# luoao-kddi/SCP

Hardware: AMD Instinct MI355X
Metric: KITTI frames/sec encode (SCP-EHEM, level 16) + bpp match vs ref (higher is better)
Workload: dtype f32 (dense layers and attention as bf16x3 split on bf16 MFMA, feature kNN as f16x3 split on f16 MFMA, fp32 accumulate; position kNN / CDF in fp32); 1 GPU; SCP-EHEM KITTI-like synthetic 120k-pt frames, --spher --mullevel lidar_level=16 (BASELINE.json configs[2]), seeded random weights; nodes_per_frame=577403, windows_per_frame=100, frames_per_gpu=46, frames_in_flight=4, frames_per_launch_sequence=1, transform=host-numpy on a prefetch thread (strict identity: the reference's integers), parallelism=frame-sharded x1, rank_cores=256, rank_cores_pinned=False

## Files before the change

include/scp.h:

```cpp
#ifndef SCP_H
#define SCP_H
#include <stddef.h>
#include <stdint.h>

#ifdef __cplusplus
extern "C" {
#endif

#define SCP_API __attribute__((visibility("default")))

#define SCP_OK 0
#define SCP_EINVAL (-1)
#define SCP_ENOMEM (-2)
#define SCP_ESMALL (-3)
#define SCP_EHIP (-4)
#define SCP_ESTATE (-5)

#define SCP_MAX_DEPTH 21
#define SCP_MAX_SEGMENTS 62

#define SCP_ABI_VERSION 220
SCP_API int scp_version(void);
SCP_API int scp_last_hip_error(void);
SCP_API int scp_device_count(void);
// ... 260 lines not shown
typedef struct scp_expand_seg {
    int64_t first, count, cfirst, coded;
    int32_t L, shift, lv_next, lv_clamp, polar, reserved;
    double mn, den;
} scp_expand_seg;
SCP_API int scp_decode_expand_batch(const int64_t *sym, const int64_t *cum, const int32_t *pos, const uint8_t *anc, const uint8_t *octant,
                                    int64_t n, const scp_expand_seg *seg, int32_t S, int32_t cs, const int64_t *wbase, int32_t K, int64_t M,
                                    int64_t T, void *table_dev, int32_t *cpos, uint8_t *canc, uint8_t *coct, uint8_t *cctx, float *cposn,
                                    uint8_t *occ8, void *stream);

SCP_API int scp_swin_ln_linear(const float *x, int64_t ldx, const float *valid, const void *Whi, const void *Wlo, const float *bias,
                               const float *wbeta, float eps, float *out, int64_t ldo, int32_t M, int32_t N, void *stream);
SCP_API int scp_swin_post_attn(const void *Ohi, const void *Olo, int64_t ldo_in, const float *x, int64_t ldx, const void *W, const float *bp,
                               const float *b1, const float *b2, float eps, float *out, int64_t ldc, int32_t M, const int32_t *tile_list,
                               int32_t n_tiles, void *stream);
SCP_API int64_t scp_swin_post_attn_weight_bytes(void);
SCP_API double scp_gelu_prescale(void);

SCP_API int scp_swin_merge(const float *x, int64_t ldx, int64_t n_src, const int64_t *ia, const int64_t *ib, const void *W, const float *wbeta,
                           float eps, float *out, int64_t ldo, int32_t M, void *stream);

SCP_API int scp_geo_edge_mlps(const float *pos1, int64_t ld1, const float *pos2, int64_t ld2, const float *pos3, int64_t ld3, const void *W,
                              const float *bias, float *out, int64_t ldo, int32_t M, void *stream);
SCP_API int scp_mlp3_rows(const float *x, int64_t ldx, int64_t n_src, const int64_t *in_map, const void *W, const float *bias, float *out, int64_t ldo,
                          const int64_t *out_map, int32_t M, int32_t N, void *stream);

SCP_API int scp_swin_kv_planes(const float *k, const float *v, int64_t ldkv, int64_t rows, void *khi, void *klo, void *vthi, void *vtlo, void *stream);
SCP_API int scp_swin_ln_qkv(const float *x, int64_t ldx, const float *valid, const void *Whi, const void *Wlo, const float *bias, const float *wbeta,
                            float eps, float *q, int64_t ldq, void *planes, int64_t Tp, int32_t M, int32_t N, void *stream);
SCP_API int scp_swin_attention_packed_planes(const float *q, const void *khi, const void *klo, const void *vthi, const void *vtlo,
// ... 8 lines not shown
```

scp_amd/csrc/rc_common.h:

```cpp
#pragma once
#include "scp_internal.h"

typedef __bf16 rbf16x8 __attribute__((ext_vector_type(8)));
typedef float rf32x16 __attribute__((ext_vector_type(16)));
typedef float rf32x4 __attribute__((ext_vector_type(4)));
typedef int ri32x4 __attribute__((ext_vector_type(4)));
typedef __attribute__((address_space(3))) void *rc_lds_ptr_t;
typedef const __attribute__((address_space(1))) void *rc_glb_ptr_t;

#define RC_ROWS 128
#define RC_BOUNCE 4096

__device__ __forceinline__ void rc_dma16(const void *g, char *l) {
    __builtin_amdgcn_global_load_lds((rc_glb_ptr_t)g, (rc_lds_ptr_t)l, 16, 0, 0);
}

typedef float rf32x2 __attribute__((ext_vector_type(2)));
typedef __bf16 rbf16x2 __attribute__((ext_vector_type(2)));
typedef unsigned ru32x4 __attribute__((ext_vector_type(4)));
typedef unsigned ru32x2 __attribute__((ext_vector_type(2)));
__device__ __forceinline__ unsigned rc_pack2(float a, float b) {
    const rf32x2 v = {a, b};
    return __builtin_bit_cast(unsigned, __builtin_convertvector(v, rbf16x2));
}
__device__ __forceinline__ void rc_split2(float a, float b, unsigned &hi, unsigned &lo) {
    asm volatile("" : "+v"(a), "+v"(b));
    hi = rc_pack2(a, b);
    lo = rc_pack2(a - __builtin_bit_cast(float, hi << 16), b - __builtin_bit_cast(float, hi & 0xffff0000u));
}
__device__ __forceinline__ void rc_split8(const float *f, rbf16x8 &hi, rbf16x8 &lo) {
    ru32x4 h, l;
#pragma unroll
    for (int i = 0; i < 4; ++i) { unsigned a, b; rc_split2(f[2 * i], f[2 * i + 1], a, b); h[i] = a; l[i] = b; }
    hi = __builtin_bit_cast(rbf16x8, h);
    lo = __builtin_bit_cast(rbf16x8, l);
}

struct RcLane {
    int lane, col, h, w;
    int frag;
    int rg;
};

// ... 57 lines not shown
```

scp_amd/csrc/rowchain.hip:

```cpp
#include <stdlib.h>
#include "scp_internal.h"
#include "rc_common.h"

#define RC_SLOT 32768
#define RC_RING (4 * RC_SLOT)
#define RC_OFF_BOUNCE RC_RING
#define RC_OFF_BIAS (RC_RING + 4 * RC_BOUNCE)
#define RC_LDS (RC_OFF_BIAS + 16384)

__device__ __forceinline__ void rc_issue_rowchunk(const RcLane &L, const __bf16 *Whi, const __bf16 *Wlo, int g, char *slot) {
#pragma unroll
    for (int j = 0; j < 4; ++j) {
        const int p = L.w + 4 * j;
        const int64_t off = ((int64_t)g * 16 + p) * 512 + L.lane * 8;
        rc_dma16(Whi + off, slot + p * 1024);
        rc_dma16(Wlo + off, slot + 16384 + p * 1024);
    }
}

__device__ __forceinline__ void rc_issue_kchunk(const RcLane &L, const __bf16 *Whi, const __bf16 *Wlo, int c, int nks, char *slot) {
#pragma unroll
    for (int j = 0; j < 4; ++j) {
        const int p = L.w + 4 * j;
        const int64_t off = ((int64_t)p * nks + c) * 512 + L.lane * 8;
// ... 556 lines not shown
            if (RC_DMA_HERE(s, gap) && RC_PROBE_DMA_ON) rc_dma_piece(L, wr, RC_DMA_SLOT(s, gap) ? n1 : n0, nxt + RC_DMA_SLOT(s, gap) * RC_SLOT, RC_DMA_IDX(s, gap), RC_DMA_PLANE(s, gap));
            if (HAS_GELU) {
                const int k = s >> 1, st = (s & 1) * 6 + gap;
                unsigned wh = 0, wl = 0;
                rc_gelu_stage(st, g, a1g[2 * k], a1g[2 * k + 1], wh, wl);
                if (st == 10) Hnh[k >> 2][k & 3] = wh;
                if (st == 11) Hnl[k >> 2][k & 3] = wl;
            }
            RC_SB;
        }
    }
    if (NEXT == 0) RC_DS_READ4_WAIT(A[0][1], fn.r0, 16384, A[0][3], fn.k0, RC_SLOT + 16384, A[0][0], fn.r0, 0, A[0][2], fn.k0, RC_SLOT);
    else RC_DS_READ4_WAIT(A[0][1], fn.r0, 16384, A[0][3], fn.r0, RC_SLOT + 16384, A[0][0], fn.r0, 0, A[0][2], fn.r0, RC_SLOT);
}

__global__ __launch_bounds__(256, 1) void rc_post_attn_kernel(const RcPostArgs a) {
    extern __shared__ __attribute__((aligned(1024))) char smem[];
    const RcLane L = rc_lane();
    const int ntiles = (a.M + RC_ROWS - 1) / RC_ROWS;
    float *sbp = (float *)(smem + RC_OFF_BIAS), *sb2 = sbp + 256, *sb1 = sbp + 512;
    for (int i = threadIdx.x; i < 256; i += 256) { sbp[i] = a.bp[i]; sb2[i] = a.b2[i]; }
    for (int i = threadIdx.x; i < 1024; i += 256) sb1[i] = a.b1[i];
    __syncthreads();
    const int nlist = a.tile_list ? a.n_list : ntiles;
    auto tile_of = [&](int i) { return a.tile_list ? a.tile_list[i] : i; };
    int ti = blockIdx.x;
    if (ti >= nlist) return;
    int tile = tile_of(ti);
    char *bounce = smem + RC_OFF_BOUNCE + L.w * RC_BOUNCE;
    const int ldc_bytes = (int)(a.ldc * 4);
    const int voff = (32 * L.w + (L.lane >> 3)) * ldc_bytes + (L.lane & 7) * 16;
// ... 190 lines not shown
        load_o(tile_next);
        rc_body_step<false, true, 0>(L, smem, gstep & 1, Y, a1[0], a1[1], Hh[0], Hl[0], Hnh, Hnl, Bh, Bl, A, wr, src_2(31), src_2(31));
        ++gstep;
        rc_body_step<false, false, 1>(L, smem, gstep & 1, Y, a1[0], a1[1], Hnh, Hnl, Hh[0], Hl[0], Bh, Bl, A, wr, src_p(0), src_p(1));
        ++gstep;
        }
        stamp(t_mlp);
        asm volatile("s_waitcnt lgkmcnt(0)" ::: "memory");
        const int64_t rows_left = (int64_t)a.M - m0;
        const int64_t span = (rows_left < RC_ROWS ? rows_left : RC_ROWS) * a.ldc * 4;
#ifdef RC_EPI_NOSTORE
        const __amdgpu_buffer_rsrc_t rs = __builtin_amdgcn_make_buffer_rsrc(a.out, 0, 0, 0x00020000);
#else
        const __amdgpu_buffer_rsrc_t rs = __builtin_amdgcn_make_buffer_rsrc(a.out + (int64_t)m0 * a.ldc, 0, (int)span, 0x00020000);
#endif
#pragma unroll
        for (int b = 0; b < 8; ++b) {
            rf32x4 o[4];
#pragma unroll
            for (int q = 0; q < 4; ++q)
#pragma unroll
                for (int u = 0; u < 4; ++u) o[q][u] = Y[b][4 * q + u];
            rc_store_block(L, bounce, o, rs, ldc_bytes, voff, 32 * b);
        }
        transpose_o();
        stamp(t_epi);
        ++n_tiles;
    }
    if (DBG && L.lane == 0) {
        unsigned long long *o = a.dbg + ((size_t)blockIdx.x * 4 + L.w) * 8;
        o[0] = t_p0; o[1] = t_mlp; o[2] = t_ln; o[3] = t_epi; o[4] = n_tiles;
        o[5] = __builtin_amdgcn_s_memtime() - t_first; o[6] = __builtin_amdgcn_s_memrealtime() - r_first;
    }
    SCP_WAIT_DMA(0);
}

#ifndef RCW_D1
#define RCW_D1 4
// ... 684 lines not shown
        configured = true;
    }
    RcLnLinArgs a;
    a.x = x; a.ldx = ldx; a.valid = valid; a.Whi = (const __bf16 *)Whi; a.Wlo = (const __bf16 *)Wlo; a.bias = bias; a.wbeta = wbeta;
    a.out = q; a.ldo = q ? ldq : 256; a.M = M; a.N = N; a.eps = eps; a.probe = 0; a.dbg = nullptr;
    a.planes = (__bf16 *)planes; a.plane_bytes = Tp * 512; a.nq = N / 64 - 8;
    const int ntiles = M / RC_ROWS, ncu = rc_num_cu();
    SCP_PROF(SCP_PROF_LN_LINEAR, stream, 2.0 * M * 256.0 * N);
    if (rc_lnlin2_here(ntiles, ncu)) return scp_lnlin2_launch(a, true, ncu, (hipStream_t)stream);
    a.ngroups = rc_ll_groups(ntiles, N / 64, ncu);
    hipLaunchKernelGGL((rc_ln_linear_kernel<0, true>), dim3((unsigned)(a.ngroups > 1 ? ntiles * a.ngroups : (ntiles < ncu ? ntiles : ncu))), dim3(256), RC_LDS, (hipStream_t)stream, a);
    LAUNCH_CHECK();
    return SCP_OK;
}

extern "C" SCP_API int scp_swin_post_attn(const void *Ohi, const void *Olo, int64_t ldo_in, const float *x, int64_t ldx, const void *W, const float *bp,
                                          const float *b1, const float *b2, float eps, float *out, int64_t ldc, int32_t M, const int32_t *tile_list,
                                          int32_t n_tiles, void *stream) {
    if (!Ohi || !Olo || !x || !W || !bp || !b1 || !b2 || !out || M <= 0 || (tile_list && (n_tiles <= 0 || n_tiles > (M + RC_ROWS - 1) / RC_ROWS)) || ldo_in < 256 || (ldo_in & 7) || ldx < 256 || (ldx & 3) || ldc < 256 ||
        (ldc & 3) || (((uintptr_t)Ohi | (uintptr_t)Olo | (uintptr_t)x | (uintptr_t)out | (uintptr_t)W) & 15) ||
        (int64_t)RC_ROWS * ldc * 4 > 0x7fffffffLL)
        return SCP_EINVAL;
    static bool configured = false;
    if (!configured) {
        HIP_TRY(hipFuncSetAttribute((const void *)rc_post_attn_kernel, hipFuncAttributeMaxDynamicSharedMemorySize, RC_LDS));
        HIP_TRY(hipFuncSetAttribute((const void *)rc_post_attn_wide_kernel, hipFuncAttributeMaxDynamicSharedMemorySize, RC_LDS));
        configured = true;
    }
    RcPostArgs a;
    a.Ohi = (const __bf16 *)Ohi; a.Olo = (const __bf16 *)Olo; a.ldo_in = ldo_in; a.x = x; a.ldx = ldx; a.W = W;
    a.bp = bp; a.b1 = b1; a.b2 = b2; a.out = out; a.ldc = ldc; a.M = M; a.eps = eps;
    a.dbg = g_rc_dbg;
    { const char *e = getenv("SCP_RC_DUMP"); a.dbg_mode = e ? atoi(e) : 0; }
    a.tile_list = tile_list; a.n_list = tile_list ? n_tiles : 0;
    const int ntiles = tile_list ? n_tiles : (M + RC_ROWS - 1) / RC_ROWS;
    const int ncu = rc_num_cu();
    SCP_PROF(SCP_PROF_POST_ATTN, stream, 2.0 * (tile_list ? (double)n_tiles * RC_ROWS : (double)M) * (256.0 * 256.0 + 2.0 * 256.0 * 1024.0));
    if (rc_wide_mode() == 1 || (rc_wide_mode() < 0 && !g_rc_dbg && !a.dbg_mode && 4 * (int64_t)ntiles <= (int64_t)ncu)) {
        const int items = 4 * ntiles;
        hipLaunchKernelGGL(rc_post_attn_wide_kernel, dim3((unsigned)(items < 2 * ncu ? items : 2 * ncu)), dim3(256), RC_LDS, (hipStream_t)stream, a);
        LAUNCH_CHECK();
        return SCP_OK;
    }
    hipLaunchKernelGGL(rc_post_attn_kernel, dim3((unsigned)(ntiles < ncu ? ntiles : ncu)), dim3(256), RC_LDS, (hipStream_t)stream, a);
    LAUNCH_CHECK();
    return SCP_OK;
}

extern "C" SCP_API int64_t scp_swin_post_attn_weight_bytes(void) { return 2 * (int64_t)RC_W_PLANE; }

extern "C" SCP_API int scp_geo_edge_mlps(const float *pos1, int64_t ld1, const float *pos2, int64_t ld2, const float *pos3, int64_t ld3, const void *W,
                                         const float *bias, float *out, int64_t ldo, int32_t M, void *stream) {
    if (!pos1 || !pos2 || !pos3 || !W || !bias || !out || M <= 0 || ld1 < 64 || ld2 < 128 || ld3 < 256 || ((ld1 | ld2 | ld3) & 3) || ldo < 128 || (ldo & 3) ||
        (((uintptr_t)pos1 | (uintptr_t)pos2 | (uintptr_t)pos3 | (uintptr_t)out | (uintptr_t)W) & 15) || (int64_t)RC_ROWS * ldo * 4 > 0x7fffffffLL)
        return SCP_EINVAL;
    static bool configured = false;
    if (!configured) {
        HIP_TRY(hipFuncSetAttribute((const void *)rc_edge_mlp_kernel, hipFuncAttributeMaxDynamicSharedMemorySize, RC_LDS));
        configured = true;
    }
    RcEdgeArgs a;
// ... 46 lines not shown
```

scp_amd/models/packed.py:

```python
import numpy as np
import torch
import torch.nn.functional as F

from .. import native
from ..ops import linear_s, leaky_mlp3_s, split_cat, linear, layer_norm, leaky_mlp3, _split, derived, frozen_epoch
from .ehem import SHIFT, WINDOW, _edge_conv_packed, qkv_fused


def _ceil512(a):
    return (a + WINDOW - 1) // WINDOW * WINDOW


def _tokens(L):
    wid = torch.repeat_interleave(torch.arange(L.numel(), device=L.device), L)
    first = torch.cumsum(L, 0) - L
    return wid, torch.arange(int(L.sum()), device=L.device) - first[wid]


class StageLayout:

    def __init__(self, L):
        self.L = L
        self.Lp = _ceil512(L)
        self.base = torch.cumsum(self.Lp, 0) - self.Lp
# ... 104 lines not shown


def _block_consts(layer, cross):
    ep = frozen_epoch()
    key = "_scp_fast_x" if cross else "_scp_fast"
    fast = layer.__dict__.get(key) if ep else None
    if fast is not None and fast[0] == ep:
        return fast[1:]
    att = layer.attention.self
    out = (_rowchain_weights(layer, cross), att.relative_position_bias_table, (att.query.bias if cross else None), layer.layernorm_before.eps, layer.layernorm_after.eps)
    if ep:
        layer.__dict__[key] = (ep,) + out
    return out


def _swin_layer_rowchain(layer, x, valid, wtab, shift, query=None, tiles=None, q_pre=None):
    cross = query is not None
    w, table, qbias, eps_b, eps_a = _block_consts(layer, cross)
    v1 = None if valid is None else valid.reshape(-1)
    if native.attention_bf16x3():
        if not cross:
            q, kvp = native.swin_ln_qkv(x, w["kv"], w["b"], eps_b, v1)
        else:
            q = q_pre if q_pre is not None else native.swin_ln_linear(query, w["q"], qbias, eps_b, v1)
            _, kvp = native.swin_ln_qkv(x, w["kv"], w["b"], eps_b, v1)
        o = native.swin_attention_packed_planes(q, kvp, table, wtab, shift, split=True, valid=v1 if tiles is not None else None)
        if tiles is not None and tiles.shape[0] > 0:
            return native.swin_post_attn(o, x, w["post"], eps_a, out=x, tiles=tiles)
        return native.swin_post_attn(o, x, w["post"], eps_a)
    att, lnb = layer.attention.self, layer.layernorm_before
    if not cross:
        qkv = native.swin_ln_linear(x, w["kv"], w["b"], lnb.eps, v1)
        q, k, v = qkv[:, :256], qkv[:, 256:512], qkv[:, 512:]
    else:
        q = q_pre if q_pre is not None else native.swin_ln_linear(query, w["q"], att.query.bias, lnb.eps, v1)
        kv = native.swin_ln_linear(x, w["kv"], w["b"], lnb.eps, v1)
        k, v = kv[:, :256], kv[:, 256:]
    o = native.swin_attention_packed(q, k, v, att.relative_position_bias_table, wtab, shift, split=True)
    return native.swin_post_attn(o, x, w["post"], layer.layernorm_after.eps)


def _swin_layer(layer, x, valid, wtab, shift, query=None, tiles=None, q_pre=None):
    fc1, fc2 = layer.intermediate.dense, layer.output.dense
    if x.shape[1] != 256 or fc1.weight.shape != (1024, 256) or fc2.weight.shape != (256, 1024):
        raise native.ScpError("EHEM's Swin blocks are 256 wide with a 1024-wide MLP (configs/model/ehem.yaml); other widths are not built")
    return _swin_layer_rowchain(layer, x, valid, wtab, shift, query, tiles, q_pre)


def _merge(m, x, maps):
    ev, od = maps
    if x.shape[1] != 256 or m.reduction.weight.shape != (256, 512) or m.reduction.bias is not None:
        raise native.ScpError("SwinPatchMerging: 2 x 256 -> 256 without bias expected")
    mw = derived(m, "rowchain_merge", [m.reduction.weight, m.norm.weight, m.norm.bias],
                 lambda: native.MergeWeights(m.reduction.weight, m.norm.weight, m.norm.bias))
    return native.swin_merge(x, ev, od, mw, m.norm.eps)


def _encoder(enc, x, valids, tabs, merges, query=None, tiles=None, q_pre=None):
    hs = [x]
    for s, stage in enumerate(enc.layers):
        for b, blk in enumerate(stage.blocks):
            x = _swin_layer(blk, x, valids[s], tabs[s], SHIFT if b % 2 else 0, query, None if tiles is None else tiles[s],
                            None if q_pre is None else q_pre[s][b])
        hs.append(x)
        if s < len(enc.layers) - 1:
            x = _merge(stage.downsample, x, merges[s])
            if query is not None and q_pre is None:
                query = _merge(stage.downsample, query, merges[s])
    return hs


def _concat(hs, cmaps, extra=None):
    n = len(hs) - 1 + (1 if extra is not None else 0)
    out = native.SplitAct.empty(hs[1].shape[0], 256 * n, hs[1].device)
    native.split_rows(hs[1], out=out.cols(0, 256))
    for s in range(1, len(hs) - 1):
        native.split_rows(hs[s + 1], idx=cmaps[s - 1], out=out.cols(256 * s, 256 * (s + 1)))
    if extra is not None:
        k = len(hs) - 1
        native.split_rows(extra[0], idx=extra[1], out=out.cols(256 * k, 256 * (k + 1)))
    return out


HIER = True


FUSE2 = __import__("os").environ.get("SCP_CONCAT_FUSE2", "1")[:1] != "0"


def _concat_layer(lin, hs, parents, extra=None, grand=None, a0_pre=None):
    n = len(hs) - 1
    def build():
        W = lin.weight.detach()
        slabs = [W[:, 256 * s:256 * (s + 1)].contiguous() for s in range(n)]
        if extra is not None:
            slabs[0] = torch.cat((slabs[0], W[:, 256 * n:256 * (n + 1)]), 1).contiguous()
        return slabs
    cache = derived(lin, "slabs+" if extra is not None else "slabs", (lin.weight,), build)
    fused = FUSE2 and n >= 3 and grand is not None and native.WTILE and hs[1].shape[0] % 256 == 0
    z = None
    for s in range(n - 1, 1 if fused else 0, -1):
        z = linear_s(native.split_rows(hs[s + 1]), cache[s], None, residual=z, res_map=None if z is None else parents[s], res_first=z is not None)
    if a0_pre is not None:
        native.split_rows(hs[1], out=a0_pre.cols(0, 256))
        a0 = a0_pre
    else:
        a0 = native.split_rows(hs[1]) if extra is None else split_cat((hs[1], extra))
    if fused:
        return native.linear_split_hier2(a0, _split(cache[0]), native.split_rows(hs[2]), _split(cache[1]), parents[0], lin.bias, native.ACT_LEAKY,
                                         residual=z, res_map=grand)
    return linear_s(a0, cache[0], lin.bias, act="leaky", residual=z, res_map=None if z is None else parents[0], res_first=z is not None,
                    want="split")


def _mlp_over_concat(seq, hs, parents, extra=None, grand=None, a0_pre=None):
    a = _concat_layer(seq[0], hs, parents, extra, grand, a0_pre)
    a = linear_s(a, seq[2].weight, seq[2].bias, act="leaky", want="split")
    return linear_s(a, seq[4].weight, seq[4].bias)


CHAIN_HEADS = __import__("os").environ.get("SCP_HEADS", "chain") != "split"


def _mlp3_weights(owner, name, seq):
    return derived(owner, "mlp3_" + name, [seq[i].weight for i in (0, 2, 4)] + [seq[i].bias for i in (0, 2, 4)], lambda: native.Mlp3Weights(seq))


def _head3(model, name, a, out=None, out_map=None, ncols=None):
    seq = getattr(model, name)
    N = seq[4].weight.shape[0]
    if CHAIN_HEADS:
# ... 42 lines not shown
    pos1 = _edge_conv_packed(g.conv1, pos0, ktab, out=f2[:, :c1])
    x = leaky_mlp3(g.mlp2, x, exact=True)
    f3 = torch.empty((P0, c2 + x.shape[1]), dtype=torch.float32, device=dev)
    f3[:, c2:] = x
    pos2 = _edge_conv_packed(g.conv2, f2, ktab, out=f3[:, :c2])
    pos3 = _edge_conv_packed(g.conv3, f3, ktab, feeds_knn=False)
    nx = g.mlp3[4].weight.shape[0]
    feat = torch.empty((P0, nx + g.edge_mlp2[4].weight.shape[0]), dtype=torch.float32, device=dev)
    leaky_mlp3_s(g.mlp3, native.split_rows(x), out=feat[:, :nx])
    if (pos1.shape[1], pos2.shape[1], pos3.shape[1]) != (64, 128, 256) or feat.shape[1] - nx != 128:
        raise native.ScpError("GeoFeatGenerator: edge features of 64 / 128 / 256 channels expected (models/dgcnn.py:74-119)")
    ew = derived(g, "rowchain_edge", [l.weight for l in (g.edge_mlp1[0], g.edge_mlp1[2], g.edge_mlp1[4], g.edge_mlp2[0], g.edge_mlp2[2], g.edge_mlp2[4])] +
                 [l.bias for l in (g.edge_mlp1[0], g.edge_mlp1[2], g.edge_mlp1[4], g.edge_mlp2[0], g.edge_mlp2[2], g.edge_mlp2[4])],
                 lambda: native.EdgeMlpWeights(g.edge_mlp1, g.edge_mlp2))
    native.geo_edge_mlps(pos1, pos2, pos3, ew, feat[:, nx:])
    hs = _encoder(model.swin_self_transformer, feat, d["self_valid"], d["self_tab"], d["self_merge"], tiles=d.get("self_tiles"))
    feat_a = _mlp_over_concat(model.ancient_mlp, hs, d["self_parent"], grand=d["self_concat"][1]) if HIER else leaky_mlp3_s(model.ancient_mlp, _concat(hs, d["self_concat"]))
    Q0 = d["a1map"].shape[0]
    a1 = native.gather_rows(feat_a, d["a1map"], torch.empty((Q0, 256), dtype=torch.float32, device=dev))
    a2 = native.gather_rows(feat_a, d["a2map"], torch.empty((Q0, 256), dtype=torch.float32, device=dev))
    st = dict(a1=a1, a2=a2, pre_occ=occ_self[d["a1map"]])
    if table is not None:
        _head_to_table(model, a1, d["even_out"], table)
        return None, st
    prob1 = _head3(model, "prob_pred_mlp1", a1)
    return prob1[d["even_rows"]], st


@torch.no_grad()
def ehem_phase2_prepare(model, st, plan):
    d = plan.d
    a1, a2 = st["a1"], st["a2"]
# ... 24 lines not shown
@torch.no_grad()
def ehem_phase2_packed(model, st, plan, pre_occ=None, table=None, prep=None):
    d = plan.d
    g = model.geo_feat_generator
    a1, a2 = st["a1"], st["a2"]
    po = st["pre_occ"] if pre_occ is None else pre_occ
    lut = derived(model, "pre_occ_lut", [g.occ_enc.weight] + [model.pre_occ_mlp[i].weight for i in (0, 2, 4)] + [model.pre_occ_mlp[i].bias for i in (0, 2, 4)],
                  lambda: leaky_mlp3(model.pre_occ_mlp, g.occ_enc.weight.detach()).contiguous())
    no = lut.shape[1]
    if prep is not None:
        pre = prep["pre"]
    else:
        pre = torch.empty((a2.shape[0], no + model.pre_attn_mlp[4].weight.shape[0]), dtype=torch.float32, device=a2.device)
        _head3(model, "pre_attn_mlp", a1, out=pre[:, no:])
    native.gather_rows(lut, po, pre[:, :no])
    hc = _encoder(model.swin_cross_transformer, pre, d["cross_valid"], d["cross_tab"], d["cross_merge"], query=a2, tiles=d.get("cross_tiles"),
                  q_pre=None if prep is None else prep["q"])
    if table is not None:
        a = _concat_layer(model.prob_pred_mlp2[0], hc, d["cross_parent"], a2, d["cross_concat"][1], None if prep is None else prep.get("a0")) if HIER else linear_s(_concat(hc, d["cross_concat"], extra=(a2, None)), model.prob_pred_mlp2[0].weight, model.prob_pred_mlp2[0].bias, act="leaky", want="split")
        from ..ops import _split
        a = linear_s(a, model.prob_pred_mlp2[2].weight, model.prob_pred_mlp2[2].bias, act="leaky", want="split")
        native.linear_split_scatter(a, _split(model.prob_pred_mlp2[4].weight), model.prob_pred_mlp2[4].bias, d["odd_out"], table)
        return None
    prob2 = (_mlp_over_concat(model.prob_pred_mlp2, hc, d["cross_parent"], extra=a2, grand=d["cross_concat"][1], a0_pre=None if prep is None else prep.get("a0")) if HIER
             else leaky_mlp3_s(model.prob_pred_mlp2, _concat(hc, d["cross_concat"], extra=(a2, None))))
    return prob2[d["odd_rows"]]


@torch.no_grad()
def ehem_forward_packed(model, ctx, pos, plan, table=None):
    ev, st = ehem_phase1_packed(model, ctx, pos, plan, table=table)
    return ev, ehem_phase2_packed(model, st, plan, table=table)
```

scp_amd/native.py:

```python
import ctypes as C
import os

import numpy as np
import torch

HERE = os.path.dirname(os.path.abspath(__file__))
LIB_PATH = os.path.join(HERE, "libscp_hip.so")
MAX_DEPTH = 21

CART, SPHER, CYLIN = 0, 1, 2
POS_MINMAX, POS_MINMAX_MUL, POS_POW2 = 0, 1, 2
_ERR = {-1: "SCP_EINVAL", -2: "SCP_ENOMEM", -3: "SCP_ESMALL", -4: "SCP_EHIP", -5: "SCP_ESTATE"}


class ScpError(RuntimeError):
    pass


class QuantInfo(C.Structure):
    _fields_ = [("bin_num", C.c_double), ("qs", C.c_double * 3), ("offset", C.c_double * 3),
                ("max_coord", C.c_int32), ("min_coord", C.c_int32)]


class Segment(C.Structure):
# ... 91 lines not shown
        "scp_octattn_attention_f16x3": (C.c_int, [_vp, _vp, _vp, _vp, _vp, i64, i32, i32, i32, i32, _vp, _vp, _vp, i64, _vp]),
        "scp_octattn_attention_rowinv": (C.c_int, [_vp, i64, i64, _vp, _vp, i64, i64, _vp, _vp, i64, i64, _vp, _vp, i64, i64, i32, i32, i32, i32, i32,
                                                   i32, _vp]),
        "scp_octattn_attention_rowinv_step": (C.c_int, [_vp, i64, _vp, _vp, i64, i64, i32, i32, _vp, _vp, i64, _vp, _vp, i64, _vp, _vp, i32, i32, i32,
                                                        _vp]),
        "scp_decode_expand_octattn": (C.c_int, [_vp, _vp, _vp, _vp, i64, i32, i32, i32, _vp, _vp, _vp, _vp, _vp]),
        "scp_decode_expand_batch": (C.c_int, [_vp, _vp, _vp, _vp, _vp, i64, _vp, i32, i32, _vp, i32, i64, i64, _vp, _vp, _vp, _vp, _vp, _vp, _vp, _vp]),
        "scp_split_weight_bf16": (C.c_int, [_vp, i32, i32, i32, i32, _vp, _vp, _vp]),
        "scp_linear_bf16x3": (C.c_int, [_vp, i64, _vp, _vp, i32, _vp, _vp, i64, _vp, i64, i32, i32, i32, i32, _vp]),
        "scp_split_weight_f16": (C.c_int, [_vp, i32, i32, i32, i32, _vp, _vp, _vp, _vp]),
        "scp_linear_f16x3": (C.c_int, [_vp, i64, _vp, _vp, _vp, i32, _vp, _vp, i64, _vp, i64, i32, i32, i32, i32, _vp, _vp]),
        "scp_linear_split": (C.c_int, [_vp, _vp, i64, _vp, _vp, i32, i32, _vp, _vp, i64, _vp, i64, _vp, _vp, i64, i32, i32, i32, i32, i32, _vp]),
        "scp_tile_weight_bf16": (C.c_int, [_vp, i32, i32, _vp, _vp]),
        "scp_swin_ln_linear": (C.c_int, [_vp, i64, _vp, _vp, _vp, _vp, _vp, C.c_float, _vp, i64, i32, i32, _vp]),
        "scp_swin_post_attn": (C.c_int, [_vp, _vp, i64, _vp, i64, _vp, _vp, _vp, _vp, C.c_float, _vp, i64, i32, _vp, i32, _vp]),
        "scp_swin_post_attn_weight_bytes": (C.c_int64, []),
        "scp_gelu_prescale": (C.c_double, []),
        "scp_split_rows": (C.c_int, [_vp, i64, i64, _vp, i32, _vp, _vp, i64, i64, _vp]),
        "scp_linear_split_scatter": (C.c_int, [_vp, _vp, i64, _vp, _vp, i32, i32, _vp, _vp, _vp, i64, i32, i32, i32, i32, i32, _vp]),
        "scp_linear_split_gather": (C.c_int, [_vp, _vp, i64, _vp, _vp, i32, i32, _vp, _vp, i64, _vp, _vp, i64, _vp, _vp, i64, i32, i32, i32, i32, i32, _vp]),
        "scp_linear_split_hier2": (C.c_int, [_vp, _vp, i64, i32, _vp, _vp, i64, i64, _vp, _vp, _vp, _vp, i32, _vp, _vp, _vp, i64, _vp, _vp, _vp, i64, i32, i32, i32, _vp]),
        "scp_layernorm_rows": (C.c_int, [_vp, i64, i64, _vp, _vp, i32, _vp, _vp, _vp, C.c_float, _vp, i64, i64, _vp]),
        "scp_layernorm_rows_split": (C.c_int, [_vp, i64, i64, _vp, _vp, i32, _vp, _vp, _vp, C.c_float, _vp, _vp, i64, i64, _vp]),
        "scp_gather_rows": (C.c_int, [_vp, i64, _vp, i32, _vp, i64, i64, _vp]),
        "scp_linear_f32": (C.c_int, [_vp, i64, _vp, _vp, _vp, i64, i32, i32, i32, i32, _vp]),
        "scp_softmax_cdf": (C.c_int, [_vp, i64, i64, i32, _vp, _vp, _vp, _vp, _vp]),
        "scp_pmf_cdf": (C.c_int, [_vp, i64, i32, _vp, _vp, _vp, _vp]),
        "scp_rate_workspace_bytes": (C.c_int64, [i64, i32]),
        "scp_rate_segments": (C.c_int, [_vp, i64, i64, i32, _vp, _vp, _vp, i32, _vp, _vp, _vp, _vp, i64, _vp]),
        "scp_nn_error_split_f64": (C.c_int, [_vp, i64, _vp, i64, _vp, _vp, i32, _vp, i32, _vp, _vp, _vp, _vp, _vp, _vp]),
# ... 1050 lines not shown
        w1d = w1.detach().double()
        s = float(lib().scp_gelu_prescale())
        swp = SplitWeight(wp.detach().float().contiguous())
        sw1 = SplitWeight((w1d * gamma.detach().double()[None, :] * s).float()[:, perm_k].contiguous())
        sw2 = SplitWeight((w2.detach().double() / s).float()[:, perm_h].contiguous())
        tiles = [_tiled_planes_always(w) for w in (swp, sw1, sw2)]
        self.packed = torch.cat([t[0].reshape(-1) for t in tiles] + [t[1].reshape(-1) for t in tiles]).contiguous()
        if self.packed.numel() * 2 != lib().scp_swin_post_attn_weight_bytes():
            raise ScpError("swin_post_attn: 256 -> 1024 -> 256 blocks only")
        self.bp = bp.detach().float().contiguous()
        self.b1 = ((b1.detach().double() + w1d @ beta.detach().double()) * s).float().contiguous()
        self.b2 = b2.detach().float().contiguous()
        note_cache_fill()


def swin_post_attn(o, x, pw, eps=1e-5, out=None, tiles=None):
    M = x.shape[0]
    if o.K != 256 or o.M != M or x.shape[1] != 256 or x.stride(1) != 1:
        raise ScpError("swin_post_attn: [M, 256] operands expected")
    if out is None:
        out = torch.empty((M, 256), dtype=torch.float32, device=x.device)
    t = o.t
    rc = lib().scp_swin_post_attn(t[0].data_ptr(), t[1].data_ptr(), t.stride(1), x.data_ptr(), x.stride(0), pw.packed.data_ptr(), _dev(pw.bp),
                                  _dev(pw.b1), _dev(pw.b2), float(eps), out.data_ptr(), out.stride(0), M,
                                  None if tiles is None else _dev(tiles, torch.int32), 0 if tiles is None else int(tiles.shape[0]), _stream())
    _check(rc, "scp_swin_post_attn")
    return out


def layernorm_rows(x, gamma, beta, eps=1e-5, valid=None, ia=None, ib=None, out=None, split=False):
    Cc = gamma.shape[0]
    rows = x.shape[0] if ia is None else ia.shape[0]
    if split:
        o = SplitAct.empty(rows, Cc, x.device)
        rc = lib().scp_layernorm_rows_split(x.data_ptr(), x.stride(0), x.shape[0], None if ia is None else _dev(ia, torch.int64),
                                            None if ib is None else _dev(ib, torch.int64), Cc, _dev(gamma), _dev(beta),
                                            None if valid is None else _dev(valid, torch.float32), float(eps), o.t[0].data_ptr(),
                                            o.t[1].data_ptr(), o.t.stride(1), rows, _stream())
        _check(rc, "scp_layernorm_rows_split")
        return o
    if out is None:
# ... 472 lines not shown
```

Before: 16.02 frames/s.

## Emit bf16 hi/lo planes from post-attention epilogue for concat MLP inputs

The last block of each Swin stage now writes its output as bf16 hi/lo split planes directly from the post-attention kernel epilogue, in addition to the fp32 rows. The hierarchical concat MLP then consumes these planes instead of launching separate split_rows kernels that re-read each stage output. The change adds extra plane stores, and zero-fill for skipped tiles, to the epilogue. In wide mode it falls back to a separate split kernel.

```diff
diff --git a/include/scp.h b/include/scp.h
--- a/include/scp.h
+++ b/include/scp.h
@@ -298,6 +298,9 @@
 SCP_API int scp_swin_post_attn(const void *Ohi, const void *Olo, int64_t ldo_in, const float *x, int64_t ldx, const void *W, const float *bp,
                                const float *b1, const float *b2, float eps, float *out, int64_t ldc, int32_t M, const int32_t *tile_list,
                                int32_t n_tiles, void *stream);
+SCP_API int scp_swin_post_attn_planes(const void *Ohi, const void *Olo, int64_t ldo_in, const float *x, int64_t ldx, const void *W, const float *bp,
+                                      const float *b1, const float *b2, float eps, float *out, int64_t ldc, int32_t M, const int32_t *tile_list,
+                                      int32_t n_tiles, void *hi, void *lo, int64_t ldp, void *stream);
 SCP_API int64_t scp_swin_post_attn_weight_bytes(void);
 SCP_API double scp_gelu_prescale(void);
 
diff --git a/scp_amd/csrc/rc_common.h b/scp_amd/csrc/rc_common.h
--- a/scp_amd/csrc/rc_common.h
+++ b/scp_amd/csrc/rc_common.h
@@ -27,6 +27,10 @@
     asm volatile("" : "+v"(a), "+v"(b));
     hi = rc_pack2(a, b);
     lo = rc_pack2(a - __builtin_bit_cast(float, hi << 16), b - __builtin_bit_cast(float, hi & 0xffff0000u));
+}
+__device__ __forceinline__ unsigned rc_split_pair(float x0, float x1, int plane) {
+    const unsigned hh = rc_pack2(x0, x1);
+    return plane ? rc_pack2(x0 - __builtin_bit_cast(float, hh << 16), x1 - __builtin_bit_cast(float, hh & 0xffff0000u)) : hh;
 }
 __device__ __forceinline__ void rc_split8(const float *f, rbf16x8 &hi, rbf16x8 &lo) {
     ru32x4 h, l;
diff --git a/scp_amd/csrc/rowchain.hip b/scp_amd/csrc/rowchain.hip
--- a/scp_amd/csrc/rowchain.hip
+++ b/scp_amd/csrc/rowchain.hip
@@ -594,7 +594,43 @@
     else RC_DS_READ4_WAIT(A[0][1], fn.r0, 16384, A[0][3], fn.r0, RC_SLOT + 16384, A[0][0], fn.r0, 0, A[0][2], fn.r0, RC_SLOT);
 }
 
-__global__ __launch_bounds__(256, 1) void rc_post_attn_kernel(const RcPostArgs a) {
+struct RcPlaneDst { __bf16 *hi, *lo; int64_t ldp; };
+
+__device__ __forceinline__ void rc_store_planes(const RcLane &L, char *bounce, const rf32x16 &c0, const rf32x16 &c1, __amdgpu_buffer_rsrc_t rhi,
+                                                __amdgpu_buffer_rsrc_t rlo, int ldp_bytes, int pvoff, int ch0) {
+    ri32x4 y[2][4];
+#pragma unroll
+    for (int plane = 0; plane < 2; ++plane) {
+#pragma unroll
+        for (int b = 0; b < 2; ++b)
+#pragma unroll
+            for (int q = 0; q < 4; ++q) {
+                const rf32x16 &c = b ? c1 : c0;
+                *(ru32x2 *)(bounce + L.col * 128 + (((4 * b + q) ^ (L.col & 7)) << 4) + 8 * L.h) =
+                    (ru32x2){rc_split_pair(c[4 * q], c[4 * q + 1], plane), rc_split_pair(c[4 * q + 2], c[4 * q + 3], plane)};
+            }
+        asm volatile("s_waitcnt lgkmcnt(0)" ::: "memory");
+#pragma unroll
+        for (int it = 0; it < 4; ++it) {
+            const int rho = 8 * it + (L.lane >> 3), kap = L.lane & 7;
+            y[plane][it] = *(const ri32x4 *)(bounce + rho * 128 + ((kap ^ (rho & 7)) << 4));
+        }
+        asm volatile("s_waitcnt lgkmcnt(0)" ::: "memory");
+    }
+#pragma unroll
+    for (int plane = 0; plane < 2; ++plane)
+#pragma unroll
+        for (int it = 0; it < 4; ++it) __builtin_amdgcn_raw_buffer_store_b128(y[plane][it], plane ? rlo : rhi, pvoff, it * 8 * ldp_bytes + ch0 * 2, 0);
+}
+
+__device__ __forceinline__ __amdgpu_buffer_rsrc_t rc_plane_rsrc(__bf16 *base, int64_t ldp, int M, int t) {
+    const int m0 = t * RC_ROWS;
+    const int rows = M - m0 < RC_ROWS ? M - m0 : RC_ROWS;
+    return __builtin_amdgcn_make_buffer_rsrc(base + (int64_t)m0 * ldp, 0, rows > 0 ? (int)((rows - 1) * ldp * 2 + 512) : 0, 0x00020000);
+}
+
+template <bool PLANES>
+__global__ __launch_bounds__(256, 1) void rc_post_attn_kernel(const RcPostArgs a, const RcPlaneDst pd_arg) {
     extern __shared__ __attribute__((aligned(1024))) char smem[];
     const RcLane L = rc_lane();
     const int ntiles = (a.M + RC_ROWS - 1) / RC_ROWS;
@@ -815,6 +851,14 @@
 #else
         const __amdgpu_buffer_rsrc_t rs = __builtin_amdgcn_make_buffer_rsrc(a.out + (int64_t)m0 * a.ldc, 0, (int)span, 0x00020000);
 #endif
+        RcPlaneDst pd = {nullptr, nullptr, 0};
+        if (PLANES) {
+            static_assert(sizeof(RcPostArgs) % 8 == 0, "the second kernel argument follows the first without padding");
+            const char __attribute__((address_space(4))) *kp = (const char __attribute__((address_space(4))) *)__builtin_amdgcn_kernarg_segment_ptr();
+            asm volatile("" : "+s"(kp));
+            const RcPlaneDst __attribute__((address_space(4))) *src = (const RcPlaneDst __attribute__((address_space(4))) *)(kp + sizeof(RcPostArgs));
+            pd.hi = src->hi; pd.lo = src->lo; pd.ldp = src->ldp;
+        }
 #pragma unroll
         for (int b = 0; b < 8; ++b) {
             rf32x4 o[4];
@@ -823,6 +867,30 @@
 #pragma unroll
                 for (int u = 0; u < 4; ++u) o[q][u] = Y[b][4 * q + u];
             rc_store_block(L, bounce, o, rs, ldc_bytes, voff, 32 * b);
+            if (PLANES && (b & 1)) {
+                const int ldp_bytes = (int)(pd.ldp * 2);
+                rc_store_planes(L, bounce, Y[b - 1], Y[b], rc_plane_rsrc(pd.hi, pd.ldp, a.M, tile), rc_plane_rsrc(pd.lo, pd.ldp, a.M, tile), ldp_bytes,
+                                (32 * L.w + (L.lane >> 3)) * ldp_bytes + (L.lane & 7) * 16, 32 * (b - 1));
+            }
+        }
+        if (PLANES && a.tile_list) {
+            const ri32x4 zero = {0, 0, 0, 0};
+            const int ldp_bytes = (int)(pd.ldp * 2);
+            const int pvoff = (32 * L.w + (L.lane >> 3)) * ldp_bytes + (L.lane & 7) * 16;
+            const int last = ti + 1 == nlist;
+            for (int side = 0; side <= last; ++side) {
+                const int g0 = side ? tile + 1 : (ti > 0 ? tile_of(ti - 1) + 1 : 0), g1 = side ? ntiles : tile;
+                for (int g = g0; g < g1; ++g) {
+                    const __amdgpu_buffer_rsrc_t zh = rc_plane_rsrc(pd.hi, pd.ldp, a.M, g), zl = rc_plane_rsrc(pd.lo, pd.ldp, a.M, g);
+#pragma unroll
+                    for (int it = 0; it < 4; ++it)
+#pragma unroll
+                        for (int p = 0; p < 4; ++p) {
+                            __builtin_amdgcn_raw_buffer_store_b128(zero, zh, pvoff, it * 8 * ldp_bytes + p * 128, 0);
+                            __builtin_amdgcn_raw_buffer_store_b128(zero, zl, pvoff, it * 8 * ldp_bytes + p * 128, 0);
+                        }
+                }
+            }
         }
         transpose_o();
         stamp(t_epi);
@@ -1537,16 +1605,18 @@
     return SCP_OK;
 }
 
-extern "C" SCP_API int scp_swin_post_attn(const void *Ohi, const void *Olo, int64_t ldo_in, const float *x, int64_t ldx, const void *W, const float *bp,
-                                          const float *b1, const float *b2, float eps, float *out, int64_t ldc, int32_t M, const int32_t *tile_list,
-                                          int32_t n_tiles, void *stream) {
+static int rc_post_attn_launch(const void *Ohi, const void *Olo, int64_t ldo_in, const float *x, int64_t ldx, const void *W, const float *bp,
+                               const float *b1, const float *b2, float eps, float *out, int64_t ldc, int32_t M, const int32_t *tile_list,
+                               int32_t n_tiles, void *Phi, void *Plo, int64_t ldp, void *stream) {
     if (!Ohi || !Olo || !x || !W || !bp || !b1 || !b2 || !out || M <= 0 || (tile_list && (n_tiles <= 0 || n_tiles > (M + RC_ROWS - 1) / RC_ROWS)) || ldo_in < 256 || (ldo_in & 7) || ldx < 256 || (ldx & 3) || ldc < 256 ||
         (ldc & 3) || (((uintptr_t)Ohi | (uintptr_t)Olo | (uintptr_t)x | (uintptr_t)out | (uintptr_t)W) & 15) ||
         (int64_t)RC_ROWS * ldc * 4 > 0x7fffffffLL)
         return SCP_EINVAL;
+    if (Phi && (ldp < 256 || (ldp & 7) || (((uintptr_t)Phi | (uintptr_t)Plo) & 15) || (int64_t)RC_ROWS * ldp * 2 > 0x7fffffffLL)) return SCP_EINVAL;
     static bool configured = false;
     if (!configured) {
-        HIP_TRY(hipFuncSetAttribute((const void *)rc_post_attn_kernel, hipFuncAttributeMaxDynamicSharedMemorySize, RC_LDS));
+        HIP_TRY(hipFuncSetAttribute((const void *)rc_post_attn_kernel<false>, hipFuncAttributeMaxDynamicSharedMemorySize, RC_LDS));
+        HIP_TRY(hipFuncSetAttribute((const void *)rc_post_attn_kernel<true>, hipFuncAttributeMaxDynamicSharedMemorySize, RC_LDS));
         HIP_TRY(hipFuncSetAttribute((const void *)rc_post_attn_wide_kernel, hipFuncAttributeMaxDynamicSharedMemorySize, RC_LDS));
         configured = true;
     }
@@ -1558,16 +1628,35 @@
     a.tile_list = tile_list; a.n_list = tile_list ? n_tiles : 0;
     const int ntiles = tile_list ? n_tiles : (M + RC_ROWS - 1) / RC_ROWS;
     const int ncu = rc_num_cu();
-    SCP_PROF(SCP_PROF_POST_ATTN, stream, 2.0 * (tile_list ? (double)n_tiles * RC_ROWS : (double)M) * (256.0 * 256.0 + 2.0 * 256.0 * 1024.0));
-    if (rc_wide_mode() == 1 || (rc_wide_mode() < 0 && !g_rc_dbg && !a.dbg_mode && 4 * (int64_t)ntiles <= (int64_t)ncu)) {
-        const int items = 4 * ntiles;
-        hipLaunchKernelGGL(rc_post_attn_wide_kernel, dim3((unsigned)(items < 2 * ncu ? items : 2 * ncu)), dim3(256), RC_LDS, (hipStream_t)stream, a);
+    const bool wide = rc_wide_mode() == 1 || (rc_wide_mode() < 0 && !g_rc_dbg && !a.dbg_mode && 4 * (int64_t)ntiles <= (int64_t)ncu);
+    {
+        SCP_PROF(SCP_PROF_POST_ATTN, stream, 2.0 * (tile_list ? (double)n_tiles * RC_ROWS : (double)M) * (256.0 * 256.0 + 2.0 * 256.0 * 1024.0));
+        if (wide) {
+            const int items = 4 * ntiles;
+            hipLaunchKernelGGL(rc_post_attn_wide_kernel, dim3((unsigned)(items < 2 * ncu ? items : 2 * ncu)), dim3(256), RC_LDS, (hipStream_t)stream, a);
+        } else {
+            const RcPlaneDst pd = {(__bf16 *)Phi, (__bf16 *)Plo, ldp};
+            const dim3 grid((unsigned)(ntiles < ncu ? ntiles : ncu));
+            if (Phi) hipLaunchKernelGGL(rc_post_attn_kernel<true>, grid, dim3(256), RC_LDS, (hipStream_t)stream, a, pd);
+            else hipLaunchKernelGGL(rc_post_attn_kernel<false>, grid, dim3(256), RC_LDS, (hipStream_t)stream, a, pd);
+        }
         LAUNCH_CHECK();
-        return SCP_OK;
-    }
-    hipLaunchKernelGGL(rc_post_attn_kernel, dim3((unsigned)(ntiles < ncu ? ntiles : ncu)), dim3(256), RC_LDS, (hipStream_t)stream, a);
-    LAUNCH_CHECK();
+    }
+    if (wide && Phi) return scp_split_rows(out, ldc, M, nullptr, 256, Phi, Plo, ldp, M, stream);
     return SCP_OK;
+}
+
+extern "C" SCP_API int scp_swin_post_attn(const void *Ohi, const void *Olo, int64_t ldo_in, const float *x, int64_t ldx, const void *W, const float *bp,
+                                          const float *b1, const float *b2, float eps, float *out, int64_t ldc, int32_t M, const int32_t *tile_list,
+                                          int32_t n_tiles, void *stream) {
+    return rc_post_attn_launch(Ohi, Olo, ldo_in, x, ldx, W, bp, b1, b2, eps, out, ldc, M, tile_list, n_tiles, nullptr, nullptr, 0, stream);
+}
+
+extern "C" SCP_API int scp_swin_post_attn_planes(const void *Ohi, const void *Olo, int64_t ldo_in, const float *x, int64_t ldx, const void *W,
+                                                 const float *bp, const float *b1, const float *b2, float eps, float *out, int64_t ldc, int32_t M,
+                                                 const int32_t *tile_list, int32_t n_tiles, void *hi, void *lo, int64_t ldp, void *stream) {
+    if (!hi || !lo) return SCP_EINVAL;
+    return rc_post_attn_launch(Ohi, Olo, ldo_in, x, ldx, W, bp, b1, b2, eps, out, ldc, M, tile_list, n_tiles, hi, lo, ldp, stream);
 }
 
 extern "C" SCP_API int64_t scp_swin_post_attn_weight_bytes(void) { return 2 * (int64_t)RC_W_PLANE; }
diff --git a/scp_amd/models/packed.py b/scp_amd/models/packed.py
--- a/scp_amd/models/packed.py
+++ b/scp_amd/models/packed.py
@@ -142,7 +142,7 @@
     return out
 
 
-def _swin_layer_rowchain(layer, x, valid, wtab, shift, query=None, tiles=None, q_pre=None):
+def _swin_layer_rowchain(layer, x, valid, wtab, shift, query=None, tiles=None, q_pre=None, planes=None):
     cross = query is not None
     w, table, qbias, eps_b, eps_a = _block_consts(layer, cross)
     v1 = None if valid is None else valid.reshape(-1)
@@ -154,8 +154,8 @@
             _, kvp = native.swin_ln_qkv(x, w["kv"], w["b"], eps_b, v1)
         o = native.swin_attention_packed_planes(q, kvp, table, wtab, shift, split=True, valid=v1 if tiles is not None else None)
         if tiles is not None and tiles.shape[0] > 0:
-            return native.swin_post_attn(o, x, w["post"], eps_a, out=x, tiles=tiles)
-        return native.swin_post_attn(o, x, w["post"], eps_a)
+            return native.swin_post_attn(o, x, w["post"], eps_a, out=x, tiles=tiles, planes=planes)
+        return native.swin_post_attn(o, x, w["post"], eps_a, planes=planes)
     att, lnb = layer.attention.self, layer.layernorm_before
     if not cross:
         qkv = native.swin_ln_linear(x, w["kv"], w["b"], lnb.eps, v1)
@@ -165,14 +165,14 @@
         kv = native.swin_ln_linear(x, w["kv"], w["b"], lnb.eps, v1)
         k, v = kv[:, :256], kv[:, 256:]
     o = native.swin_attention_packed(q, k, v, att.relative_position_bias_table, wtab, shift, split=True)
-    return native.swin_post_attn(o, x, w["post"], layer.layernorm_after.eps)
-
-
-def _swin_layer(layer, x, valid, wtab, shift, query=None, tiles=None, q_pre=None):
+    return native.swin_post_attn(o, x, w["post"], layer.layernorm_after.eps, planes=planes)
+
+
+def _swin_layer(layer, x, valid, wtab, shift, query=None, tiles=None, q_pre=None, planes=None):
     fc1, fc2 = layer.intermediate.dense, layer.output.dense
     if x.shape[1] != 256 or fc1.weight.shape != (1024, 256) or fc2.weight.shape != (256, 1024):
         raise native.ScpError("EHEM's Swin blocks are 256 wide with a 1024-wide MLP (configs/model/ehem.yaml); other widths are not built")
-    return _swin_layer_rowchain(layer, x, valid, wtab, shift, query, tiles, q_pre)
+    return _swin_layer_rowchain(layer, x, valid, wtab, shift, query, tiles, q_pre, planes)
 
 
 def _merge(m, x, maps):
@@ -184,18 +184,26 @@
     return native.swin_merge(x, ev, od, mw, m.norm.eps)
 
 
-def _encoder(enc, x, valids, tabs, merges, query=None, tiles=None, q_pre=None):
-    hs = [x]
+STAGE_PLANES = __import__("os").environ.get("SCP_STAGE_PLANES", "1")[:1] != "0"
+
+
+def _encoder(enc, x, valids, tabs, merges, query=None, tiles=None, q_pre=None, want_planes=False, plane0=None):
+    hs, pl = [x], [None]
     for s, stage in enumerate(enc.layers):
+        last = len(stage.blocks) - 1
         for b, blk in enumerate(stage.blocks):
+            dst = None
+            if want_planes and b == last:
+                dst = plane0 if (s == 0 and plane0 is not None) else native.SplitAct.empty(x.shape[0], 256, x.device)
+                pl.append(dst)
             x = _swin_layer(blk, x, valids[s], tabs[s], SHIFT if b % 2 else 0, query, None if tiles is None else tiles[s],
-                            None if q_pre is None else q_pre[s][b])
+                            None if q_pre is None else q_pre[s][b], dst)
         hs.append(x)
         if s < len(enc.layers) - 1:
             x = _merge(stage.downsample, x, merges[s])
             if query is not None and q_pre is None:
                 query = _merge(stage.downsample, query, merges[s])
-    return hs
+    return (hs, pl) if want_planes else hs
 
 
 def _concat(hs, cmaps, extra=None):
@@ -216,8 +224,9 @@
 FUSE2 = __import__("os").environ.get("SCP_CONCAT_FUSE2", "1")[:1] != "0"
 
 
-def _concat_layer(lin, hs, parents, extra=None, grand=None, a0_pre=None):
+def _concat_layer(lin, hs, parents, extra=None, grand=None, a0_pre=None, pl=None):
     n = len(hs) - 1
+    planes_of = (lambda k: pl[k]) if pl is not None else (lambda k: native.split_rows(hs[k]))
     def build():
         W = lin.weight.detach()
         slabs = [W[:, 256 * s:256 * (s + 1)].contiguous() for s in range(n)]
@@ -228,21 +237,22 @@
     fused = FUSE2 and n >= 3 and grand is not None and native.WTILE and hs[1].shape[0] % 256 == 0
     z = None
     for s in range(n - 1, 1 if fused else 0, -1):
-        z = linear_s(native.split_rows(hs[s + 1]), cache[s], None, residual=z, res_map=None if z is None else parents[s], res_first=z is not None)
+        z = linear_s(planes_of(s + 1), cache[s], None, residual=z, res_map=None if z is None else parents[s], res_first=z is not None)
     if a0_pre is not None:
-        native.split_rows(hs[1], out=a0_pre.cols(0, 256))
+        if pl is None:
+            native.split_rows(hs[1], out=a0_pre.cols(0, 256))
         a0 = a0_pre
     else:
-        a0 = native.split_rows(hs[1]) if extra is None else split_cat((hs[1], extra))
+        a0 = planes_of(1) if extra is None else split_cat((hs[1], extra))
     if fused:
-        return native.linear_split_hier2(a0, _split(cache[0]), native.split_rows(hs[2]), _split(cache[1]), parents[0], lin.bias, native.ACT_LEAKY,
+        return native.linear_split_hier2(a0, _split(cache[0]), planes_of(2), _split(cache[1]), parents[0], lin.bias, native.ACT_LEAKY,
                                          residual=z, res_map=grand)
     return linear_s(a0, cache[0], lin.bias, act="leaky", residual=z, res_map=None if z is None else parents[0], res_first=z is not None,
                     want="split")
 
 
-def _mlp_over_concat(seq, hs, parents, extra=None, grand=None, a0_pre=None):
-    a = _concat_layer(seq[0], hs, parents, extra, grand, a0_pre)
+def _mlp_over_concat(seq, hs, parents, extra=None, grand=None, a0_pre=None, pl=None):
+    a = _concat_layer(seq[0], hs, parents, extra, grand, a0_pre, pl)
     a = linear_s(a, seq[2].weight, seq[2].bias, act="leaky", want="split")
     return linear_s(a, seq[4].weight, seq[4].bias)
 
@@ -315,8 +325,12 @@
                  [l.bias for l in (g.edge_mlp1[0], g.edge_mlp1[2], g.edge_mlp1[4], g.edge_mlp2[0], g.edge_mlp2[2], g.edge_mlp2[4])],
                  lambda: native.EdgeMlpWeights(g.edge_mlp1, g.edge_mlp2))
     native.geo_edge_mlps(pos1, pos2, pos3, ew, feat[:, nx:])
-    hs = _encoder(model.swin_self_transformer, feat, d["self_valid"], d["self_tab"], d["self_merge"], tiles=d.get("self_tiles"))
-    feat_a = _mlp_over_concat(model.ancient_mlp, hs, d["self_parent"], grand=d["self_concat"][1]) if HIER else leaky_mlp3_s(model.ancient_mlp, _concat(hs, d["self_concat"]))
+    pl = None
+    if HIER and STAGE_PLANES:
+        hs, pl = _encoder(model.swin_self_transformer, feat, d["self_valid"], d["self_tab"], d["self_merge"], tiles=d.get("self_tiles"), want_planes=True)
+    else:
+        hs = _encoder(model.swin_self_transformer, feat, d["self_valid"], d["self_tab"], d["self_merge"], tiles=d.get("self_tiles"))
+    feat_a = _mlp_over_concat(model.ancient_mlp, hs, d["self_parent"], grand=d["self_concat"][1], pl=pl) if HIER else leaky_mlp3_s(model.ancient_mlp, _concat(hs, d["self_concat"]))
     Q0 = d["a1map"].shape[0]
     a1 = native.gather_rows(feat_a, d["a1map"], torch.empty((Q0, 256), dtype=torch.float32, device=dev))
     a2 = native.gather_rows(feat_a, d["a2map"], torch.empty((Q0, 256), dtype=torch.float32, device=dev))
@@ -371,15 +385,23 @@
         pre = torch.empty((a2.shape[0], no + model.pre_attn_mlp[4].weight.shape[0]), dtype=torch.float32, device=a2.device)
         _head3(model, "pre_attn_mlp", a1, out=pre[:, no:])
     native.gather_rows(lut, po, pre[:, :no])
-    hc = _encoder(model.swin_cross_transformer, pre, d["cross_valid"], d["cross_tab"], d["cross_merge"], query=a2, tiles=d.get("cross_tiles"),
-                  q_pre=None if prep is None else prep["q"])
+    a0_pre, pl = None if prep is None else prep.get("a0"), None
+    if HIER and STAGE_PLANES:
+        if a0_pre is None:
+            a0_pre = native.SplitAct.empty(a2.shape[0], 512, a2.device)
+            native.split_rows(a2, out=a0_pre.cols(256, 512))
+        hc, pl = _encoder(model.swin_cross_transformer, pre, d["cross_valid"], d["cross_tab"], d["cross_merge"], query=a2, tiles=d.get("cross_tiles"),
+                          q_pre=None if prep is None else prep["q"], want_planes=True, plane0=a0_pre.cols(0, 256))
+    else:
+        hc = _encoder(model.swin_cross_transformer, pre, d["cross_valid"], d["cross_tab"], d["cross_merge"], query=a2, tiles=d.get("cross_tiles"),
+                      q_pre=None if prep is None else prep["q"])
     if table is not None:
-        a = _concat_layer(model.prob_pred_mlp2[0], hc, d["cross_parent"], a2, d["cross_concat"][1], None if prep is None else prep.get("a0")) if HIER else linear_s(_concat(hc, d["cross_concat"], extra=(a2, None)), model.prob_pred_mlp2[0].weight, model.prob_pred_mlp2[0].bias, act="leaky", want="split")
+        a = _concat_layer(model.prob_pred_mlp2[0], hc, d["cross_parent"], a2, d["cross_concat"][1], a0_pre, pl) if HIER else linear_s(_concat(hc, d["cross_concat"], extra=(a2, None)), model.prob_pred_mlp2[0].weight, model.prob_pred_mlp2[0].bias, act="leaky", want="split")
         from ..ops import _split
         a = linear_s(a, model.prob_pred_mlp2[2].weight, model.prob_pred_mlp2[2].bias, act="leaky", want="split")
         native.linear_split_scatter(a, _split(model.prob_pred_mlp2[4].weight), model.prob_pred_mlp2[4].bias, d["odd_out"], table)
         return None
-    prob2 = (_mlp_over_concat(model.prob_pred_mlp2, hc, d["cross_parent"], extra=a2, grand=d["cross_concat"][1], a0_pre=None if prep is None else prep.get("a0")) if HIER
+    prob2 = (_mlp_over_concat(model.prob_pred_mlp2, hc, d["cross_parent"], extra=a2, grand=d["cross_concat"][1], a0_pre=a0_pre, pl=pl) if HIER
              else leaky_mlp3_s(model.prob_pred_mlp2, _concat(hc, d["cross_concat"], extra=(a2, None))))
     return prob2[d["odd_rows"]]
 
diff --git a/scp_amd/native.py b/scp_amd/native.py
--- a/scp_amd/native.py
+++ b/scp_amd/native.py
@@ -129,6 +129,7 @@
         "scp_tile_weight_bf16": (C.c_int, [_vp, i32, i32, _vp, _vp]),
         "scp_swin_ln_linear": (C.c_int, [_vp, i64, _vp, _vp, _vp, _vp, _vp, C.c_float, _vp, i64, i32, i32, _vp]),
         "scp_swin_post_attn": (C.c_int, [_vp, _vp, i64, _vp, i64, _vp, _vp, _vp, _vp, C.c_float, _vp, i64, i32, _vp, i32, _vp]),
+        "scp_swin_post_attn_planes": (C.c_int, [_vp, _vp, i64, _vp, i64, _vp, _vp, _vp, _vp, C.c_float, _vp, i64, i32, _vp, i32, _vp, _vp, i64, _vp]),
         "scp_swin_post_attn_weight_bytes": (C.c_int64, []),
         "scp_gelu_prescale": (C.c_double, []),
         "scp_split_rows": (C.c_int, [_vp, i64, i64, _vp, i32, _vp, _vp, i64, i64, _vp]),
@@ -1209,17 +1210,23 @@
         note_cache_fill()
 
 
-def swin_post_attn(o, x, pw, eps=1e-5, out=None, tiles=None):
+def swin_post_attn(o, x, pw, eps=1e-5, out=None, tiles=None, planes=None):
     M = x.shape[0]
     if o.K != 256 or o.M != M or x.shape[1] != 256 or x.stride(1) != 1:
         raise ScpError("swin_post_attn: [M, 256] operands expected")
     if out is None:
         out = torch.empty((M, 256), dtype=torch.float32, device=x.device)
     t = o.t
-    rc = lib().scp_swin_post_attn(t[0].data_ptr(), t[1].data_ptr(), t.stride(1), x.data_ptr(), x.stride(0), pw.packed.data_ptr(), _dev(pw.bp),
-                                  _dev(pw.b1), _dev(pw.b2), float(eps), out.data_ptr(), out.stride(0), M,
-                                  None if tiles is None else _dev(tiles, torch.int32), 0 if tiles is None else int(tiles.shape[0]), _stream())
-    _check(rc, "scp_swin_post_attn")
+    args = (t[0].data_ptr(), t[1].data_ptr(), t.stride(1), x.data_ptr(), x.stride(0), pw.packed.data_ptr(), _dev(pw.bp),
+            _dev(pw.b1), _dev(pw.b2), float(eps), out.data_ptr(), out.stride(0), M,
+            None if tiles is None else _dev(tiles, torch.int32), 0 if tiles is None else int(tiles.shape[0]))
+    if planes is None:
+        _check(lib().scp_swin_post_attn(*args, _stream()), "scp_swin_post_attn")
+        return out
+    p = planes.t
+    if planes.K != 256 or planes.M != M or p.dtype != torch.bfloat16 or p.stride(2) != 1 or p.device != x.device:
+        raise ScpError("swin_post_attn: planes must be a bfloat16 SplitAct [M, 256] on the rows' device")
+    _check(lib().scp_swin_post_attn_planes(*args, p[0].data_ptr(), p[1].data_ptr(), p.stride(1), _stream()), "scp_swin_post_attn_planes")
     return out
 
 
```

New measurement: 16.16 frames/s, median of 6. No clear change (+0.9%).
